# zxhuang1698/ShapeClipper

Measured on AMD Instinct MI355X. Metric: train-step images/sec (Pix3D cfg, bs32/GPU), higher is better.
Workload: dtype f32 (bf16x3-split MFMA, fp32 accumulate)

## Files before the change

include/shapeclipper_hip.h:

```cpp
#ifndef SHAPECLIPPER_HIP_H
#define SHAPECLIPPER_HIP_H
#include <stdint.h>
#ifdef __cplusplus
extern "C" {
#endif

int sc_chamfer3d_forward(const float* xyz1, const float* xyz2, float* dist1, float* dist2,
                         int32_t* idx1, int32_t* idx2, int b, int n, int m, void* stream);

int sc_chamfer3d_forward_split(const float* xyz1, const float* xyz2, float* dist1, float* dist2,
                               int32_t* idx1, int32_t* idx2, int b, int n, int m, int nsplit,
                               void* workspace, void* stream);

long long sc_chamfer3d_grid_workspace_bytes(int b, int n, int m);
int sc_chamfer3d_forward_grid(const float* xyz1, const float* xyz2, float* dist1, float* dist2,
                              int32_t* idx1, int32_t* idx2, int b, int n, int m, void* workspace, void* stream);

int sc_chamfer3d_backward(const float* xyz1, const float* xyz2, float* gradxyz1, float* gradxyz2,
                          const float* graddist1, const float* graddist2, const int32_t* idx1,
                          const int32_t* idx2, int b, int n, int m, void* stream);

long long sc_chamfer3d_backward_ordered_workspace_bytes(int b, int n, int m);
int sc_chamfer3d_backward_ordered_chunk(void);
int sc_chamfer3d_backward_ordered(const float* xyz1, const float* xyz2, float* gradxyz1, float* gradxyz2,
// ... 359 lines not shown
                            const float* flip_elev, const float* flip_theta, int n_images, float elev_lo, float elev_hi,
                            float theta_lo, float theta_hi, float margin_eps, int emd_p, float* out, float* grads,
                            void* stream);
int sc_camera_prior_backward(const float* grads, int n_images, const float* G_margin, const float* G_uniform,
                             const float* G_sym, float* g_azim, float* g_elev, float* g_theta, float* g_flip_azim,
                             float* g_flip_elev, float* g_flip_theta, void* stream);

int sc_transform_normal_forward(const float* normals, const float* pose, int n_images, int n_per_image, float* out,
                                void* stream);
int sc_transform_normal_backward(const float* normals, const float* g_out, int n_images, int n_per_image, float* g_pose,
                                 void* stream);

int sc_loss_total_forward(const float* const* values, const float* weights, int n_terms, float* total, unsigned char* bad,
                          void* stream);
int sc_loss_total_backward(const float* weights, int n_terms, const float* G, float* g_values, void* stream);

long long sc_conv3x3_pack_floats(int cin, int cout, int hw);
long long sc_conv3x3_workspace_floats(int hw);
int sc_conv3x3_tile_channels(int hw);
int sc_conv3x3_pack_multi(const long long* table, int n, float* dst, long long total, void* stream);
int sc_conv3x3_pack_multi_units(const long long* table, int n, float* dst, long long total, void* stream);
int sc_conv3x3_pack(const float* w, float* w_pack, int cin, int cout, int hw, int transpose_flip, void* stream);
int sc_conv3x3_forward(const float* x, const float* w_pack, float* out, float* workspace, int batch, int cin, int cout, int hw,
                       void* stream);

long long sc_conv3x3_pack_floats_split(int cin, int cout, int hw);
long long sc_conv3x3_workspace_floats_split(int hw);
int sc_conv3x3_tile_channels_split(int hw);
int sc_conv3x3_forward_split(const float* x, const float* w_pack, float* out, float* workspace, int batch, int cin, int cout, int hw,
                             void* stream);
int sc_conv3x3_forward_add(const float* x, const float* w_pack, const float* addend, float* out, float* workspace, int batch, int cin,
                           int cout, int hw, int split, void* stream);

long long sc_conv3x3s2_bd_pack_floats(int cin, int cout, int hw);
long long sc_conv3x3s2_bd_workspace_floats(int hw);
int sc_conv3x3s2_bd_pack(const float* w, float* w_pack, int cin, int cout, int hw, void* stream);
int sc_conv3x3s2_backward_data(const float* gy, const float* w_pack, float* gx, float* workspace, int batch, int cin, int cout, int hw,
                               void* stream);
int sc_conv3x3s2_wgrad(const float* gy, const float* x, float* dw, float* workspace, int batch, int cin, int cout, int hw, void* stream);
long long sc_conv3x3s2_pack_floats(int cin, int cout, int hw);
long long sc_conv3x3s2_workspace_floats(int hw);
int sc_conv3x3s2_forward(const float* x, const float* w_pack, float* out, float* workspace, int batch, int cin, int cout, int hw,
                         void* stream);

long long sc_conv3x3_wgrad_workspace_floats(int cin, int cout);
int sc_conv3x3_wgrad(const float* gy, const float* x, float* dw, float* workspace, int batch, int cin, int cout, int hw, void* stream);
int sc_conv3x3_wgrad_split(const float* gy, const float* x, float* dw, float* workspace, int batch, int cin, int cout, int hw, void* stream);

long long sc_conv_stem_wgrad_workspace_floats(void);
int sc_conv_stem_forward(const float* x, const float* w, float* out, int batch, void* stream);
int sc_conv_stem_wgrad(const float* gy, const float* x, float* dw, float* workspace, int batch, void* stream);

long long sc_conv1x1s2_wgrad_workspace_floats(int cin, int cout);
int sc_conv1x1s2_forward(const float* x, const float* w, float* out, int batch, int cin, int cout, int hin, void* stream);
int sc_conv1x1s2_backward_data(const float* gy, const float* w, float* gx, int batch, int cin, int cout, int hin, void* stream);
int sc_conv1x1s2_wgrad(const float* gy, const float* x, float* dw, float* workspace, int batch, int cin, int cout, int hin, void* stream);

typedef struct sc_block_args {
    const float *x, *pf1, *pf2, *pb1, *pb2;
    const float *g1, *b1, *g2, *b2;
    float *rm1, *rv1, *rm2, *rv2;
    int64_t *nt1, *nt2;
    float *y1, *a1, *y2, *out, *st1, *st2;
    float *conv_ws, *bn_ws, *wgrad_ws;
    const float* d_out;
    float *dy2, *dres, *da1, *dy1, *dx, *gw1, *gw2, *dgb1, *dgb2;
// ... 67 lines not shown
```

shapeclipper_amd/_lib.py:

```python
from __future__ import annotations

import ctypes
import os
import re
import threading
from typing import Optional

import torch

_HERE = os.path.dirname(os.path.abspath(__file__))
LIB_PATH = os.environ.get("SHAPECLIPPER_HIP_LIB") or os.path.join(_HERE, "lib", "libshapeclipper_hip.so")

HEADER_PATH = os.path.join(_HERE, os.pardir, "include", "shapeclipper_hip.h")
_CTYPES = {"int": ctypes.c_int, "long long": ctypes.c_longlong, "float": ctypes.c_float, "double": ctypes.c_double}


def read_signatures(text):
    text = re.sub(r"/\*.*?\*/|//[^\n]*", " ", text, flags=re.S)
    text = re.sub(r"^[ \t]*#.*$", " ", text, flags=re.M)
    text = re.sub(r"typedef struct sc_block_args \{.*?\} sc_block_args", " ", text, flags=re.S)
    text = re.sub(r'extern "C" \{|\}', " ", text)
    sigs = {}
    for decl in filter(None, (" ".join(d.split()) for d in text.split(";"))):
        m = re.fullmatch(r"(int|long long) (sc_\w+)\((.*)\)", decl)
        if m is None:
            raise RuntimeError("shapeclipper_amd: include/shapeclipper_hip.h: unrecognised declaration %r" % decl)
        params = [] if m.group(3) == "void" else m.group(3).split(",")
        try:
            args = [ctypes.c_void_p if "*" in p else _CTYPES[" ".join(w for w in p.split()[:-1] if w != "const")] for p in params]
        except KeyError:
            raise RuntimeError("shapeclipper_amd: include/shapeclipper_hip.h: unrecognised parameter type in %r" % decl) from None
        sigs[m.group(2)] = (_CTYPES[m.group(1)], args)
    return sigs


with open(HEADER_PATH) as _f:
    SIGNATURES = read_signatures(_f.read())
SYMBOLS = tuple(n for n, (res, _) in SIGNATURES.items() if res is ctypes.c_int)
SYMBOLS_OTHER = tuple(n for n, (res, _) in SIGNATURES.items() if res is ctypes.c_longlong)

_lib: Optional[ctypes.CDLL] = None

TIMING = None
TIMING_SKIP = ("sc_sdf_stream_pack", "sc_sdf_stream_pack_bytes", "sc_rgb_composite_backward_fused_parts", "sc_rgb_composite_backward_fused_partial_floats", "sc_latent_bias_forward", "sc_latent_bias_backward", "sc_set_reserved_cus", "sc_grid_cus", "sc_chamfer3d_backward_ordered_chunk","sc_conv3x3_release_tables", "sc_linear_bn_supported", "sc_linear_bn_forward", "sc_linear_bn_backward", "sc_linear_backward_data", "sc_bn_splits", "sc_isosurface_blocks_per_image", "sc_marching_cubes_mesh_vertex_blocks_per_image", "sc_bn_act_forward", "sc_bn_act_backward", "sc_bn_relu_pool_forward", "sc_bn_relu_pool_backward",
               "sc_conv3x3_forward", "sc_conv3x3_forward_split", "sc_conv3x3_forward_add", "sc_conv3x3_wgrad", "sc_conv3x3_wgrad_split", "sc_conv3x3_pack", "sc_conv3x3_pack_multi", "sc_conv3x3_pack_multi_units",
               "sc_conv_stem_forward", "sc_conv_stem_wgrad", "sc_conv1x1s2_forward", "sc_conv1x1s2_backward_data", "sc_conv1x1s2_wgrad",
               "sc_conv3x3s2_forward", "sc_conv3x3s2_bd_pack", "sc_conv3x3s2_backward_data", "sc_conv3x3s2_wgrad", "sc_conv3x3_tile_channels", "sc_conv3x3_tile_channels_split",
               "sc_basic_block_forward", "sc_basic_block_backward")

class _Timed:

    def __init__(self, name, fn):
        self.name, self.fn = name, fn

    def __call__(self, *args):
        if TIMING is None:
            return self.fn(*args)
        s, e = torch.cuda.Event(enable_timing=True), torch.cuda.Event(enable_timing=True)
        s.record()
        code = self.fn(*args)
        e.record()
        TIMING.setdefault(self.name, []).append((s, e, args))
        return code


class _LibProxy:

    def __init__(self, cdll):
        self._cdll = cdll
        for name, (restype, argtypes) in SIGNATURES.items():
            fn = getattr(cdll, name)
            fn.restype, fn.argtypes = restype, argtypes
            setattr(self, name, _Timed(name, fn) if restype is ctypes.c_int and name not in TIMING_SKIP else fn)


class HipLibraryMissing(RuntimeError):
    pass


def load():
    global _lib
# ... 43 lines not shown
```

shapeclipper_amd/csrc/conv3x3.hip:

```cpp
#include <hip/hip_runtime.h>

#include <map>
#include <mutex>
#include <tuple>
#include <vector>

#include "grid_cus.hpp"
#include "shapeclipper_hip.h"

#ifndef SC_CONV_SPANS
#define SC_CONV_SPANS 1
#endif
#ifndef SC_CONV_ABLATE
#define SC_CONV_ABLATE 0
#endif

namespace sc {

#ifdef SC_CONV_PROFILE
__device__ unsigned long long* conv_prof_buf = nullptr;
#define CV_STAMP(ID) { const unsigned long long t_ = __builtin_amdgcn_s_memrealtime(); if (conv_prof_buf && tid == 0) conv_prof_buf[(size_t)g * 32 + (ID)] = t_; }
#else
#define CV_STAMP(ID)
#endif

typedef float f32x16 __attribute__((ext_vector_type(16)));
typedef __bf16 cv_bf16x8 __attribute__((ext_vector_type(8)));
typedef __bf16 cv_bf16x2 __attribute__((ext_vector_type(2)));
typedef __attribute__((address_space(3))) void* lptr_cv_t;

__device__ __forceinline__ void conv_glds16(const void* gsrc, unsigned lds_dst) {
    unsigned keep;
    asm volatile("s_mov_b32 %0, m0\n\ts_mov_b32 m0, %2\n\ts_nop 0\n\tglobal_load_lds_dwordx4 %1, off\n\ts_mov_b32 m0, %0"
                 : "=&s"(keep) : "v"(gsrc), "s"(lds_dst) : "memory");
}

template <int W_, int CT_, int PT_, int WGM_, int WGN_, bool SPLIT_ = false, int S_ = 1, bool BD2_ = false>
struct ConvCfg {
    static constexpr int W = W_, CT = CT_, PT = PT_, WGM = WGM_, WGN = WGN_, CB = 8;
// ... 436 lines not shown
        for (int i = 0; i < C::WM; ++i)
#pragma unroll
            for (int j = 0; j < C::WN; ++j) {
                const float4 v = src[(((wave * C::WM + i) * C::WN + j) * 4 + (r0 >> 2)) * 64 + lane];
                acc[i][j][0] += v.x; acc[i][j][1] += v.y; acc[i][j][2] += v.z; acc[i][j][3] += v.w;
            }
    }
    const int tile = sp.rounds * G + t;
    int phase, pt, ct;
    conv_tile_decode<C>(tile, nct, phase, pt, ct);
#pragma unroll
    for (int j = 0; j < C::WN; ++j) {
        const int p = pt * C::PT + (wn * C::WN + j) * 32 + (lane & 31);
        if (p >= npix) continue;
        int cs;
        float* ob = conv_out_pixel<C>(out, p, phase, cout, cs);
#pragma unroll
        for (int i = 0; i < C::WM; ++i)
#pragma unroll
            for (int r = 0; r < 4; ++r) {
                const int co = ct * C::CT + (wm * C::WM + i) * 32 + r + 2 * r0 + 4 * (lane >> 5);
                if (co < cout) ob[(size_t)co * cs] = addend ? acc[i][j][r] + addend[(ob - out) + (size_t)co * cs] : acc[i][j][r];
            }
    }
#ifdef SC_CONV_PROFILE
    asm volatile("s_waitcnt vmcnt(0)" ::: "memory");
    if (conv_prof_buf && tid == 0) conv_prof_buf[(size_t)(8192 + blockIdx.x * 4 + blockIdx.y) * 2 + 1] = __builtin_amdgcn_s_memrealtime();
#endif
}

__device__ __forceinline__ float conv_w_at(const float* __restrict__ w, int cin, int cout, int co, int ci, int tap, int transpose_flip) {
    return transpose_flip ? w[((size_t)ci * cout + co) * 9 + (8 - tap)] : w[((size_t)co * cin + ci) * 9 + tap];
}
__device__ __forceinline__ unsigned conv_bf16_piece(float v, int pc) {
    const __bf16 h0 = (__bf16)v;
    const float r1 = v - (float)h0;
    const __bf16 h1 = (__bf16)r1;
    const __bf16 h2 = (__bf16)(r1 - (float)h1);
    const __bf16 h = pc == 0 ? h0 : pc == 1 ? h1 : h2;
    return (unsigned)__builtin_bit_cast(unsigned short, h);
}
__device__ __forceinline__ float conv_pack_word(const float* __restrict__ w, unsigned t, int CT, int nk, int cin, int cout, int flip,
                                                bool split) {
    if (!split) {
        const int s4 = (int)(t & 3);
        t >>= 2;
        const int cl = (int)(t % CT);
        t /= CT;
        const int h = (int)(t & 1);
        t >>= 1;
        const int tap = (int)(t % 9);
        t /= 9;
        const int kb = (int)(t % nk), ct = (int)(t / nk);
        const int ci = kb * 8 + 4 * h + s4, co = ct * CT + cl;
        return co < cout ? conv_w_at(w, cin, cout, co, ci, tap, flip) : 0.f;
    }
    const int wi = (int)(t & 3);
    t >>= 2;
    const int cl = (int)(t % CT);
    t /= CT;
    const int h = (int)(t & 1);
    t >>= 1;
    const int pc = (int)(t % 3);
    t /= 3;
    const int slot = (int)(t % 9);
    t /= 9;
    const int nkp = (nk + 1) >> 1, kp = (int)(t % nkp), ct = (int)(t / nkp);
    const int kb = 2 * kp + (slot < 4 ? 0 : (slot < 8 ? 1 : h)), tap = slot < 8 ? 2 * (slot & 3) + h : 8;
    const int co = ct * CT + cl, ci = kb * 8 + 2 * wi;
    unsigned lo = 0, hi = 0;
    if (kb < nk && co < cout) {
        lo = conv_bf16_piece(conv_w_at(w, cin, cout, co, ci, tap, flip), pc);
        hi = conv_bf16_piece(conv_w_at(w, cin, cout, co, ci + 1, tap, flip), pc);
    }
// ... 46 lines not shown
using Conv56S = ConvCfg<56, 64, 512, 1, 8, true>;
using Conv28S = ConvCfg<28, 64, 512, 1, 8, true>;
using Conv14S = ConvCfg<14, 64, 512, 1, 8, true>;
using Conv7S = ConvCfg<7, 64, 256, 1, 8, true>;
using Conv28BD = ConvCfg<28, 64, 512, 1, 8, true, 1, true>;
using Conv14BD = ConvCfg<14, 64, 512, 1, 8, true, 1, true>;
using Conv7BD = ConvCfg<7, 64, 256, 1, 8, true, 1, true>;

template <class C>
static long long pack_floats(int cin, int cout) {
    if (cin % C::CB) return -1;
    const long long nct = (cout + C::CT - 1) / C::CT, nk = cin / C::CB;
    return C::PAIRED ? nct * ((nk + 1) / 2) * 9 * C::PSZ : nct * nk * C::WIMG;
}

__global__ void conv3x3_pack_multi_kernel(const long long* __restrict__ table_g, int n, float* __restrict__ dst, long long total) {
    __shared__ long long table[128 * 6];
    for (int i = threadIdx.x; i < n * 6; i += blockDim.x) table[i] = table_g[i];
    __syncthreads();
    for (long long i = (long long)blockIdx.x * blockDim.x + threadIdx.x; i < total; i += (long long)gridDim.x * blockDim.x) {
        int lo = 0, hi = n - 1;
        while (lo < hi) {
            const int mid = (lo + hi + 1) >> 1;
            if (table[mid * 6 + 1] <= i) lo = mid; else hi = mid - 1;
        }
        const long long* row = table + lo * 6;
        const float* w = reinterpret_cast<const float*>(row[0]);
        const int cin = (int)row[2], cout = (int)row[3], CT = (int)row[4], flags = (int)row[5];
        dst[i] = conv_pack_word(w, (unsigned)(i - row[1]), CT, cin / 8, cin, cout, flags & 1, (flags & 2) != 0);
    }
}

__global__ __launch_bounds__(256) void conv3x3_pack_multi_split_kernel(const long long* __restrict__ table_g, int n, float* __restrict__ dst) {
    constexpr int CT = 64, UNIT = 9 * 3 * 2 * CT * 4, LST = 145;
    __shared__ float wl[CT * LST];
    __shared__ long long row_s[6];
    const int tid = threadIdx.x;
    const long long i0 = (long long)blockIdx.x * UNIT;
    if (tid == 0) {
        int lo = 0, hi = n - 1;
        while (lo < hi) {
            const int mid = (lo + hi + 1) >> 1;
            if (table_g[mid * 6 + 1] <= i0) lo = mid; else hi = mid - 1;
        }
        for (int k = 0; k < 6; ++k) row_s[k] = table_g[lo * 6 + k];
    }
    __syncthreads();
    const float* w = reinterpret_cast<const float*>(row_s[0]);
    const int cin = (int)row_s[2], cout = (int)row_s[3], flip = (int)row_s[5] & 1, nkp = (cin / 8 + 1) / 2;
    const int unit = (int)((i0 - row_s[1]) / UNIT), ct = unit / nkp, kp = unit - ct * nkp;
    for (int e = tid; e < 16 * CT * 9; e += 256) {
        int cl, sc, tap;
        float v = 0.f;
        if (flip) {
            sc = e / (CT * 9);
            const int r = e - sc * (CT * 9);
            cl = r / 9; tap = 8 - (r - cl * 9);
            if (ct * CT + cl < cout && kp * 16 + sc < cin) v = w[((size_t)(kp * 16 + sc) * cout + ct * CT) * 9 + r];
        } else {
            cl = e / 144;
            const int r = e - cl * 144;
            sc = r / 9; tap = r - sc * 9;
            if (ct * CT + cl < cout && kp * 16 + sc < cin) v = w[((size_t)(ct * CT + cl) * cin + kp * 16) * 9 + r];
        }
        wl[cl * LST + sc * 9 + tap] = v;
    }
    __syncthreads();
    for (int v = tid; v < UNIT; v += 256) {
        const int wi = v & 3, cl = (v >> 2) & 63, h = (v >> 8) & 1, q = v >> 9, pc = q % 3, slot = q / 3;
        const int kl = slot < 4 ? 0 : (slot < 8 ? 1 : h), tap = slot < 8 ? 2 * (slot & 3) + h : 8;
        const unsigned lo = conv_bf16_piece(wl[cl * LST + (8 * kl + 2 * wi) * 9 + tap], pc);
        const unsigned hi = conv_bf16_piece(wl[cl * LST + (8 * kl + 2 * wi + 1) * 9 + tap], pc);
        dst[i0 + v] = __uint_as_float(lo | (hi << 16));
    }
}

static int conv_grid() { return grid_cus(); }

template <class C>
static long long workspace_floats() { return (long long)conv_grid() * C::WGS_PER_CU * 2 * C::TILE; }

template <class C>
static int launch_pack(const float* w, float* wpack, int cin, int cout, int tf, hipStream_t st) {
    if (cin % C::CB) return (int)hipErrorInvalidValue;
    const long long total = pack_floats<C>(cin, cout);
    hipLaunchKernelGGL((conv3x3_pack_kernel<C>), dim3((unsigned)((total + 255) / 256 < 2048 ? (total + 255) / 256 : 2048)), dim3(256), 0, st,
                       w, wpack, cin, cout, tf);
    return (int)hipGetLastError();
}

struct SpanTable {
    int* dev = nullptr;
    std::vector<int> host;
};
static std::mutex span_mu;
static std::map<std::tuple<int, int, int, int, int>, SpanTable> span_cache;

static const int* conv_spans(int tail_tiles, int nk, int G, int ov2, hipStream_t st) {
    std::map<std::tuple<int, int, int, int, int>, SpanTable>& cache = span_cache;
    int dev = 0;
    (void)hipGetDevice(&dev);
    std::lock_guard<std::mutex> lock(span_mu);
    const auto key = std::make_tuple(dev, tail_tiles, nk, G, ov2);
// ... 253 lines not shown
```

shapeclipper_amd/model/resnet.py:

```python
from __future__ import annotations

import torch
import torch.nn as nn

from ..functional import basic_block, basic_block_takes, bn_act, bn_relu_maxpool, conv1x1s2, conv3x3, conv3x3s2, conv_stem

FUSED_BN = True
HIP_CONV3X3 = True
HIP_CONV_STEM = True
HIP_CONV3X3_S2 = True
HIP_CONV3X3_S2_GRADS = True
HIP_CONV_1X1 = True
FUSED_BLOCK = True
HIP_CONV3X3_SPLIT = True


class BasicBlock(nn.Module):
    expansion = 1

    def __init__(self, inplanes, planes, stride=1, downsample=None):
        super().__init__()
        self.conv1 = nn.Conv2d(inplanes, planes, 3, stride, 1, bias=False)
        self.bn1 = nn.BatchNorm2d(planes)
        self.relu = nn.ReLU(inplace=True)
# ... 52 lines not shown
        if not FUSED_BN:
            if groups > 1:
                return torch.cat([self.forward(c) for c in x.chunk(groups)], 0)
            x = self.maxpool(self.relu(self.bn1(self.conv1(x))))
            x = self.layer4(self.layer3(self.layer2(self.layer1(x))))
        else:
            use_hip = HIP_CONV3X3 if getattr(self, "hip_conv3x3", None) is None else self.hip_conv3x3
            packs = self._conv_packs(x) if use_hip else None
            x = bn_relu_maxpool(self.bn1, conv_stem(self.conv1, x) if HIP_CONV_STEM else self.conv1(x), groups=groups)
            for layer in (self.layer1, self.layer2, self.layer3, self.layer4):
                for block in layer:
                    x = block(x, groups=groups, packs=packs, hip_conv=use_hip)
        return self.fc(torch.flatten(self.avgpool(x), 1))


def _conv_packs(self, x):
    from .. import ops
    if not (x.is_cuda and x.dtype == torch.float32 and x.shape[2] == x.shape[3]):
        return None
    key = (x.shape[2], x.device.index, HIP_CONV3X3_SPLIT)
    cache = self.__dict__.setdefault("_pack_cache", {})
    packs = cache.get(key)
    if packs is None or (packs and packs.stale()):
        side = ((x.shape[2] + 2 * 3 - 7) // 2 + 1 + 2 - 3) // 2 + 1
        items = []
        for layer in (self.layer1, self.layer2, self.layer3, self.layer4):
            for block in layer:
                if block.conv1.stride == (2, 2):
                    side = (side + 2 - 3) // 2 + 1
                for conv in ((block.conv2,) if block.conv1.stride != (1, 1) else (block.conv1, block.conv2)):
                    if ops.conv3x3_supported((1, conv.in_channels, side, side), conv.weight.shape, conv.stride, conv.padding) and conv.bias is None:
                        items.append((conv.weight, side))
        packs = cache[key] = ops.Conv3x3PackSet(items, split=HIP_CONV3X3_SPLIT) if items else False
    if packs:
        packs.refresh()
    return packs or None


ResNet._conv_packs = _conv_packs

_LAYERS = {"resnet18": [2, 2, 2, 2], "resnet34": [3, 4, 6, 3]}


def build(name: str, pretrained: bool = False, allow_random: bool = False) -> ResNet:
    if name not in _LAYERS:
        raise NotImplementedError("encoder '%s' (available: %s)" % (name, sorted(_LAYERS)))
    net = ResNet(_LAYERS[name])
    if pretrained:
        try:
            import torchvision
            state = getattr(torchvision.models, name)(pretrained=True).state_dict()
        except Exception as e:
            msg = "ImageNet weights for %s could not be loaded (%s: %s)" % (name, type(e).__name__, e)
            if not allow_random:
                raise RuntimeError(msg + "; pass --arch.enc_pretrained! to train the ResNet trunks from a random "
                                         "initialisation, or --load/--resume a checkpoint") from e
            from ..utils.util import log
            log.warn("WARNING: " + msg + " -- %s starts from a RANDOM initialisation" % name)
        else:
            net.load_state_dict(state)
    return net
```

shapeclipper_amd/model/runner.py:

```python
from __future__ import annotations

import contextlib
import importlib
import os
import shutil
import time
from copy import deepcopy

import numpy as np
import torch
import tqdm

from ..data.pix3d import sample_rays_device
from ..parallel import FlatGradAllReduce, ModuleHolder
from ..utils import eval_3D, options, util
from ..utils.util import EasyDict as edict
from ..utils.util import cleanup, log, setup

try:
    from ..utils import util_vis
except Exception:
    util_vis = None


# ... 175 lines not shown
                if cat_samples[c] >= 1:
                    continue
                cat_samples[c] += 1
                sample = {}
                for key, value in batch.items():
                    if isinstance(value, torch.Tensor):
                        sample[key] = value[i].unsqueeze(0)
                    elif isinstance(value, dict):
                        sample[key] = {k: v[i].unsqueeze(0) for k, v in value.items()}
                    else:
                        raise NotImplementedError(key)
                self.viz_data.append(sample)

    def build_networks(self, opt):
        if _rank0(opt): log.info("building networks...")
        name = "pretrainer" if opt.pretrain else "graph"
        module = importlib.import_module("shapeclipper_amd.model.{}".format(name))
        dev = torch.device("cuda", opt.device) if isinstance(opt.device, int) else torch.device(opt.device)
        reserve = int(options.hip(opt, "reserve_cus") or 0)
        if dev.type == "cuda":
            from .. import ops
            ops.set_reserved_cus(reserve if opt.world_size > 1 else 0)
        self.graph = ModuleHolder(module.Graph(opt).to(dev))
        if opt.world_size > 1:
            self.reducer = FlatGradAllReduce(self.graph.module, opt.world_size,
                                             overlap=None if options.hip(opt, "overlap_allreduce") else False)

    def setup_optimizer(self, opt):
        if _rank0(opt): log.info("setting up optimizers...")
        kwargs = {k: (tuple(v) if k == "betas" else v) for k, v in opt.optim.params.items()}
        on_gpu = next(self.graph.parameters()).is_cuda
        if on_gpu and self.optimizer in (torch.optim.Adam, torch.optim.AdamW) and options.hip(opt, "fused_adam"):
            kwargs.setdefault("fused", True)
        full, view = [], []
        for k, v in self.graph.named_parameters():
            full.append(v)
            if "estimator" in k:
                view.append(v)
        self.optim_full = self.optimizer([dict(params=full, lr=opt.optim.lr)], **kwargs)
        self.optim_V = self.optimizer([dict(params=view, lr=opt.optim.lr)], **kwargs)
        self._guarded_step = bool(kwargs.get("fused")) and bool(options.hip(opt, "guarded_step"))

    def restore_checkpoint(self, opt, best=False, evaluate=False):
        epoch_start, iter_start = None, None
        if opt.resume:
            if _rank0(opt): log.info("resuming from previous checkpoint...")
            epoch_start, iter_start, self.best_val = util.restore_checkpoint(
                opt, self, resume=opt.resume, best=best if opt.data.dataset != "openimage" else False, evaluate=evaluate)
        elif opt.load is not None:
            if _rank0(opt): log.info("loading weights from checkpoint {}...".format(opt.load))
            epoch_start, iter_start, _ = util.restore_checkpoint(opt, self, load_name=opt.load)
        elif _rank0(opt):
            log.info("initializing weights from scratch...")
        self.epoch_start = epoch_start or 0
        self.iter_start = iter_start or 0

    def setup_visualizer(self, opt):
        if _rank0(opt) and opt.tb:
            try:
                from torch.utils.tensorboard import SummaryWriter
                self.tb = SummaryWriter(log_dir=opt.output_path, flush_secs=10)
            except Exception:
                log.info("tensorboard not available; scalar logging goes to stdout only")

    def train(self, opt):
        if _rank0(opt): log.title("TRAINING START")
        self.graph.module.estimator.reset_scales()
        self.timer = edict(start=time.time(), it_mean=None)
        self.iter_skip = self.iter_start % len(self.train_loader)
        self.it = self.iter_start
        if not opt.resume:
            self.best_val, self.best_ep = np.inf, 1
        if self.iter_start == 0 and _rank0(opt) and opt.freq.eval:
# ... 709 lines not shown
```

shapeclipper_amd/ops.py:

```python
from __future__ import annotations

import collections
import ctypes
import weakref

import torch

from . import _lib
from .packing import n_tiles

_SCRATCH = {}


def _scratch(tag, dev, n_floats):
    if dev.type != "cuda":
        raise RuntimeError(_lib.NO_CPU)
    key = (tag, dev.index, torch._C._cuda_getCurrentRawStream(dev.index))
    buf = _SCRATCH.get(key)
    if buf is None or buf.numel() < n_floats:
        buf = _SCRATCH[key] = torch.empty(n_floats, device=dev, dtype=torch.float32)
    return buf


SDF_SCRATCH_FLOATS = 256 * 8 * 5 * 1024
# ... 1131 lines not shown


def conv3x3s2_backward_data(gy, w, hw):
    lib = _lib.load()
    gy, w = _aligned(gy), _aligned(w)
    B, cout = gy.shape[0], gy.shape[1]
    cin = w.shape[1]
    n = lib.sc_conv3x3s2_bd_pack_floats(cin, cout, hw)
    if n < 0 or tuple(gy.shape[2:]) != (hw // 2, hw // 2) or w.shape[0] != cout:
        raise RuntimeError("shapeclipper_amd: sc_conv3x3s2_backward_data does not take gy %s with w %s" % (tuple(gy.shape), tuple(w.shape)))
    w_pack = torch.empty(n, device=gy.device, dtype=torch.float32)
    _lib.check(lib.sc_conv3x3s2_bd_pack(_lib.ptr(w), _lib.ptr(w_pack), cin, cout, hw, _lib.stream()), "sc_conv3x3s2_bd_pack")
    ws = _scratch("conv s2bd %d" % hw, gy.device, lib.sc_conv3x3s2_bd_workspace_floats(hw))
    gx = torch.empty(B, cin, hw, hw, device=gy.device, dtype=torch.float32)
    _lib.check(lib.sc_conv3x3s2_backward_data(_lib.ptr(gy), _lib.ptr(w_pack), _lib.ptr(gx), _lib.ptr(ws), B, cin, cout, hw, _lib.stream()),
               "sc_conv3x3s2_backward_data")
    return gx


def conv3x3s2_backward_weight(gy, x):
    lib = _lib.load()
    gy, x = _aligned(gy), _aligned(x)
    B, cin, hw, _ = x.shape
    cout = gy.shape[1]
    n = lib.sc_conv3x3_wgrad_workspace_floats(cin, cout)
    if n < 0 or hw not in (56, 28, 14) or tuple(gy.shape) != (B, cout, hw // 2, hw // 2):
        raise RuntimeError("shapeclipper_amd: sc_conv3x3s2_wgrad does not take gy %s with x %s" % (tuple(gy.shape), tuple(x.shape)))
    ws = _scratch("conv wgrad", x.device, n)
    dw = torch.empty(cout, cin, 3, 3, device=x.device, dtype=torch.float32)
    _lib.check(lib.sc_conv3x3s2_wgrad(_lib.ptr(gy), _lib.ptr(x), _lib.ptr(dw), _lib.ptr(ws), B, cin, cout, hw, _lib.stream()), "sc_conv3x3s2_wgrad")
    return dw


class Conv3x3PackSet:

    def __init__(self, items, split=False):
        lib = _lib.load()
        self.split = bool(split)
        self.weights = [w for w, _ in items]
        self.ptrs = [w.data_ptr() for w in self.weights]
        rows, off, self.where = [], 0, {}
        for k, (w, side) in enumerate(items):
            if not (w.is_cuda and w.is_contiguous() and w.dtype == torch.float32):
                raise RuntimeError("shapeclipper_amd: Conv3x3PackSet needs contiguous fp32 device filters")
            for flip in (0, 1):
                cin, cout = (w.shape[0], w.shape[1]) if flip else (w.shape[1], w.shape[0])
                n = (lib.sc_conv3x3_pack_floats_split if split else lib.sc_conv3x3_pack_floats)(cin, cout, side)
                if n < 0:
                    raise RuntimeError("shapeclipper_amd: sc_conv3x3 does not take %dx%d maps with a %s filter" % (side, side, tuple(w.shape)))
                ct = (lib.sc_conv3x3_tile_channels_split if split else lib.sc_conv3x3_tile_channels)(side)
                rows.append([w.data_ptr(), off, cin, cout, ct, flip | (2 if split else 0)])
                self.where[(k, flip)] = (off, n)
                off += n
        if len(rows) > 128:
            raise RuntimeError("shapeclipper_amd: Conv3x3PackSet holds at most 64 filters (sc_conv3x3_pack_multi table limit)")
        dev = self.weights[0].device
        self.total = off
        self.units = bool(split) and all(r[4] == 64 for r in rows) and off % 13824 == 0
        self.table = torch.tensor(rows, dtype=torch.int64).to(dev)
        self.buf = torch.empty(off, device=dev, dtype=torch.float32)
        self.index = {id(w): k for k, w in enumerate(self.weights)}

    def stale(self):
        return any(w.data_ptr() != p for w, p in zip(self.weights, self.ptrs))

    def refresh(self):
        lib = _lib.load()
        fn = lib.sc_conv3x3_pack_multi_units if self.units else lib.sc_conv3x3_pack_multi
        _lib.check(fn(_lib.ptr(self.table), len(self.where), _lib.ptr(self.buf), self.total, _lib.stream()), "sc_conv3x3_pack_multi")

    def get(self, w, flip):
        off, n = self.where[(self.index[id(w)], int(flip))]
        return self.buf[off:off + n]


def linear_bn_supported(N, Cin, Cout, groups) -> bool:
    return bool(_lib.load().sc_linear_bn_supported(N, Cin, Cout, groups))


def linear_bn_forward(x, w, gamma, beta, res, running_mean, running_var, n_tracked, training, momentum, eps, relu, groups):
    N, Cin = x.shape
    Cout = w.shape[0]
    y, out = torch.empty(N, Cout, device=x.device, dtype=torch.float32), torch.empty(N, Cout, device=x.device, dtype=torch.float32)
    stats = torch.empty(2, groups, Cout, device=x.device, dtype=torch.float32)
    code = _lib.load().sc_linear_bn_forward(_lib.ptr(x), _lib.ptr(w), _lib.ptr(gamma), _lib.ptr(beta), _lib.ptr(res), _lib.ptr(y), _lib.ptr(out),
                                            _lib.ptr(stats[0]), _lib.ptr(stats[1]), _lib.ptr(running_mean), _lib.ptr(running_var), _lib.ptr(n_tracked),
                                            N, Cin, Cout, groups, 1 if training else 0, 1 if relu else 0,
                                            eps, momentum, _lib.stream())
    _lib.check(code, "sc_linear_bn_forward")
    return out, y, stats


def linear_bn_backward(g_out, gy_next, w_next, g_add, out, y, stats, gamma, x, want_res, training, relu, groups):
    N, Cin = x.shape
    Cout = y.shape[1]
    f32 = dict(device=x.device, dtype=torch.float32)
    gy = torch.empty(N, Cout, **f32)
# ... 828 lines not shown
```

shapeclipper_amd/utils/options.py:

```python
from __future__ import annotations

import collections
import importlib
import os
import random
import string
import sys

import numpy as np
import torch
import yaml

from . import util
from .util import EasyDict as edict
from .util import log

torch.backends.cudnn.benchmark = False

Switch = collections.namedtuple("Switch", ["key", "default", "kind", "text", "drives"])
HIP_TABLE = tuple(Switch(*row) for row in (
    ("device_rng", False, bool, "draw the render's jitter on the GPU (no 4 MB upload per render, another random stream than the reference)", None),
    ("device_choice", True, bool, "pick the regularisation view on the device (reg.n_views = 1)", None),
    ("device_rays", True, bool, "Pix3D: silhouette-weighted ray choice for the whole batch on the GPU (csrc/silhouette_rays.hip)", None),
    ("device_clip_preprocess", True, bool, "Pix3D: CLIP preprocessing on the GPU (csrc/clip_preprocess.hip)", None),
    ("fused_backward", True, bool, "SDF reverse pass with the weight gradients formed in the kernel (sc_sdf_backward_fused)", None),
    ("deterministic_conv", False, bool, "torch.backends.cudnn.deterministic, process-global", None),
    ("fused_loss", True, bool, "the render losses of one render in a single launch (csrc/loss.hip)", None),
    ("fused_adam", True, bool, "torch's fused Adam on the device", None),
    ("guarded_step", True, bool, "a non-finite loss skips the update on the device; the host raises one step later", None),
    ("batched_encoders", True, bool, "one grouped encoder pass and one grouped estimator pass per step", None),
    ("two_streams", True, bool, "the view estimator runs on a side stream next to the encoders", None),
    ("overlap_allreduce", False, bool, "multi-GPU: the early gradient segment is all-reduced from inside backward", None),
    ("reserve_cus", 0, (0, None), "multi-GPU: persistent convolution grids sized for the device's CUs minus this many", None),
    ("fused_block", True, bool, "one autograd node per stride-1 BasicBlock", ("model.resnet", "FUSED_BLOCK")),
    ("fused_bottleneck", True, bool, "1x1 Bottleneck_Linear blocks as fused launches (csrc/bottleneck.hip)", ("model.view_estimator", "HIP_BOTTLENECK")),
    ("fused_rgb_wgrad", True, bool, "RGB reverse pass forms the weight gradients in the kernel; off: Gy_l / r_l through HBM and sc_wgrad",
     ("ops", "FUSED_RGB_WGRAD")),
    ("rgb_stash", True, bool, "RGB forward parks its hidden activations for the reverse pass; off: the reverse pass recomputes them",
     ("ops", "RGB_STASH")),
    ("value_split", True, bool, "value-only SDF calls (evaluation grid) on the pre-split bf16x3 chain; off: fp32 MFMA", ("ops", "SDF_VALUE_SPLIT")),
    ("rgb_split", True, bool, "RGB network of the forward pass from pre-split bf16x3 fragments; off: fp32 MFMA", ("ops", "RGB_FWD_SPLIT")),
    ("rgb_bwd_split", True, bool, "RGB reverse chain from pre-split transposed fragments; off: fp32 MFMA (see HIP_REQUIRES)",
     ("ops", "RGB_BWD_SPLIT")),
    ("sdf_stream", True, bool, "SDF forward (value, feature, d sdf/dx) from streamed pre-split fragments; off: fp32 MFMA", ("ops", "SDF_FWD_STREAM")),
    ("upload_stream", True, bool, "the CPU-generator draws are copied on a stream of their own, ahead of the render",
     ("model.renderer", "UPLOAD_STREAM")),
    ("rocblas", True, bool, "the small fp32 GEMMs left to torch go through rocBLAS, process-global; off leaves torch's choice alone", None),
    ("conv3x3", True, bool, "3x3 stride-1 trunk convolutions on csrc/conv3x3.hip", ("model.resnet", "HIP_CONV3X3")),
    ("conv3x3_split", True, bool, "... as exact three-piece bf16 operand splits; off: fp32 MFMA throughout", ("model.resnet", "HIP_CONV3X3_SPLIT")),
    ("conv_stem", True, bool, "the 7x7 stride-2 stem convolution on its HIP kernel", ("model.resnet", "HIP_CONV_STEM")),
    ("conv1x1", True, bool, "the 1x1 stride-2 shortcut convolutions on their HIP kernels", ("model.resnet", "HIP_CONV_1X1")),
    ("conv3x3s2", True, bool, "the 3x3 stride-2 convolutions' forward on its HIP kernel", ("model.resnet", "HIP_CONV3X3_S2")),
    ("conv3x3s2_grads", True, bool, "... and their backward-data / weight gradient", ("model.resnet", "HIP_CONV3X3_S2_GRADS")),
    ("train_vis", False, bool, "training-time visualisation on rank 0: turn-table GIFs and periodic dumps", None),
    ("mesh_color", False, bool, "every mesh dump also writes a coloured PLY with vertex normals", None),
    ("largest_component", False, bool, "evaluation keeps the largest connected component of the level grid", None),
    ("surface_render", False, bool, "every per-sample dump also gets a render at the SDF zero crossing (Renderer.render_surface)", None),
    ("surface_refine", 3, (0, 16), "... refinement rounds of the crossing", None),
    ("surface_scale", 1, (1, 4), "... pixels per pixel side", None),
))
HIP = {row.key: row for row in HIP_TABLE}
# ... 228 lines not shown
```

Baseline: 1032.

## Fuse Adam update with conv3x3 filter repacking in one native launch

Replaces torch's fused Adam with a custom HIP kernel that updates all parameters in one launch. For conv3x3 filters it also writes the bf16x3-split packed weight images (forward and transposed) straight from the updated values. Pack sets are then marked current, so the per-step separate repack pass is skipped. The cost is a more complex pointer table with a pinned-memory upload ring, version tracking for pack staleness, and an Adam update computed in mixed double/float arithmetic that may differ slightly from torch's.

```diff
diff --git a/include/shapeclipper_hip.h b/include/shapeclipper_hip.h
--- a/include/shapeclipper_hip.h
+++ b/include/shapeclipper_hip.h
@@ -415,6 +415,9 @@
 int sc_conv3x3_forward_add(const float* x, const float* w_pack, const float* addend, float* out, float* workspace, int batch, int cin,
                            int cout, int hw, int split, void* stream);
 
+int sc_adam_step(const long long* tensors, int n_tensors, const long long* blocks, int n_blocks, const long long* chunks, int n_chunks,
+                 double lr, double beta1, double beta2, double eps, const float* found_inf, void* stream);
+
 long long sc_conv3x3s2_bd_pack_floats(int cin, int cout, int hw);
 long long sc_conv3x3s2_bd_workspace_floats(int hw);
 int sc_conv3x3s2_bd_pack(const float* w, float* w_pack, int cin, int cout, int hw, void* stream);
diff --git a/shapeclipper_amd/_lib.py b/shapeclipper_amd/_lib.py
--- a/shapeclipper_amd/_lib.py
+++ b/shapeclipper_amd/_lib.py
@@ -46,7 +46,8 @@
                "sc_conv3x3_forward", "sc_conv3x3_forward_split", "sc_conv3x3_forward_add", "sc_conv3x3_wgrad", "sc_conv3x3_wgrad_split", "sc_conv3x3_pack", "sc_conv3x3_pack_multi", "sc_conv3x3_pack_multi_units",
                "sc_conv_stem_forward", "sc_conv_stem_wgrad", "sc_conv1x1s2_forward", "sc_conv1x1s2_backward_data", "sc_conv1x1s2_wgrad",
                "sc_conv3x3s2_forward", "sc_conv3x3s2_bd_pack", "sc_conv3x3s2_backward_data", "sc_conv3x3s2_wgrad", "sc_conv3x3_tile_channels", "sc_conv3x3_tile_channels_split",
-               "sc_basic_block_forward", "sc_basic_block_backward")
+               "sc_basic_block_forward", "sc_basic_block_backward",
+               "sc_adam_step")
 
 class _Timed:
 
diff --git a/shapeclipper_amd/csrc/adam.hip b/shapeclipper_amd/csrc/adam.hip
--- /dev/null
+++ b/shapeclipper_amd/csrc/adam.hip
@@ -0,0 +1,193 @@
+#include <hip/hip_runtime.h>
+
+#include <cstdint>
+
+#include "conv_pack.hpp"
+#include "shapeclipper_hip.h"
+
+namespace sc {
+namespace adam {
+
+constexpr int THREADS = 1024, WAVES = THREADS / 64, CHUNK = 1024, TROW = 6, BROW = 8, CROW = 2;
+constexpr int FB = 64, SEG = FB * 9, LST = SEG + 1;
+constexpr int LDS_BYTES = FB * LST * 4;
+
+struct Coef {
+    float step_size, bc2_sqrt;
+    double b1, b2, eps;
+};
+
+__device__ __forceinline__ double pow_n(double b, unsigned n) {
+    double r = 1.0;
+    for (; n; n >>= 1, b *= b)
+        if (n & 1) r *= b;
+    return r;
+}
+
+__device__ __forceinline__ Coef coefficients(float step_old, double lr, double b1, double b2, double eps) {
+    const unsigned n = (unsigned)(step_old + 1.f);
+    const float bc1 = (float)(1.0 - pow_n(b1, n)), bc2_sqrt = (float)sqrt(1.0 - pow_n(b2, n));
+    return {(float)(lr / (double)bc1), bc2_sqrt, b1, b2, eps};
+}
+
+__device__ __forceinline__ void update(float& p, float g, float& m, float& v, const Coef& c) {
+    m = (float)fma(c.b1, (double)m, (1.0 - c.b1) * (double)g);
+    v = (float)fma(c.b2, (double)v, (1.0 - c.b2) * (double)g * (double)g);
+    const float denom = (float)((double)(sqrtf(v) / c.bc2_sqrt) + c.eps);
+    p -= c.step_size * m / denom;
+}
+
+__device__ __forceinline__ void update4(float4& p, const float4& g, float4& m, float4& v, const Coef& c) {
+    update(p.x, g.x, m.x, v.x, c);
+    update(p.y, g.y, m.y, v.y, c);
+    update(p.z, g.z, m.z, v.z, c);
+    update(p.w, g.w, m.w, v.w, c);
+}
+
+__device__ __forceinline__ float4 load4(const float* a, bool vec) {
+    if (vec) return *reinterpret_cast<const float4*>(a);
+    return make_float4(a[0], a[1], a[2], a[3]);
+}
+__device__ __forceinline__ void store4(float* a, const float4& x, bool vec) {
+    if (vec) {
+        *reinterpret_cast<float4*>(a) = x;
+    } else {
+        a[0] = x.x; a[1] = x.y; a[2] = x.z; a[3] = x.w;
+    }
+}
+__device__ __forceinline__ bool aligned16(const void* a, const void* b, const void* c, const void* d) {
+    return (((uintptr_t)a | (uintptr_t)b | (uintptr_t)c | (uintptr_t)d) & 15) == 0;
+}
+
+__global__ __launch_bounds__(THREADS) void adam_step_kernel(const long long* __restrict__ tensors, int n_tensors,
+                                                            const long long* __restrict__ blocks, int n_blocks,
+                                                            const long long* __restrict__ chunks, int n_chunks, double lr, double b1,
+                                                            double b2, double eps, const float* __restrict__ found_inf) {
+    extern __shared__ __attribute__((aligned(16))) float wl[];
+    const int tid = threadIdx.x;
+    const bool skip = found_inf != nullptr && *found_inf != 0.f;
+    if ((int)blockIdx.x >= n_blocks) {
+        const int wave = __builtin_amdgcn_readfirstlane(tid >> 6), lane = tid & 63;
+        const long long c = (long long)((int)blockIdx.x - n_blocks) * WAVES + wave;
+        if (skip || c >= n_chunks) return;
+        const int t = (int)chunks[c * CROW];
+        if (t < 0 || t >= n_tensors) return;
+        const long long start = chunks[c * CROW + 1];
+        const long long* tr = tensors + (size_t)t * TROW;
+        const long long left = tr[5] - start;
+        const int n = left < CHUNK ? (int)left : CHUNK;
+        float* __restrict__ p = reinterpret_cast<float*>(tr[0]) + start;
+        const float* __restrict__ g = reinterpret_cast<const float*>(tr[1]) + start;
+        float* __restrict__ m = reinterpret_cast<float*>(tr[2]) + start;
+        float* __restrict__ v = reinterpret_cast<float*>(tr[3]) + start;
+        const Coef cf = coefficients(*reinterpret_cast<const float*>(tr[4]), lr, b1, b2, eps);
+        const int nq = aligned16(p, g, m, v) ? n >> 2 : 0;
+#pragma unroll 1
+        for (int k0 = 0; k0 < 4 && 64 * k0 < nq; k0 += 2) {
+            float4 P[2], G[2], M[2], V[2];
+#pragma unroll
+            for (int k = 0; k < 2; ++k) {
+                const int q = lane + 64 * (k0 + k);
+                if (q < nq) {
+                    P[k] = load4(p + 4 * q, true); G[k] = load4(g + 4 * q, true);
+                    M[k] = load4(m + 4 * q, true); V[k] = load4(v + 4 * q, true);
+                }
+            }
+#pragma unroll
+            for (int k = 0; k < 2; ++k) {
+                const int q = lane + 64 * (k0 + k);
+                if (q < nq) {
+                    update4(P[k], G[k], M[k], V[k], cf);
+                    store4(p + 4 * q, P[k], true); store4(m + 4 * q, M[k], true); store4(v + 4 * q, V[k], true);
+                }
+            }
+        }
+        for (int e = 4 * nq + lane; e < n; e += 64) {
+            float pe = p[e], me = m[e], ve = v[e];
+            update(pe, g[e], me, ve, cf);
+            p[e] = pe; m[e] = me; v[e] = ve;
+        }
+        return;
+    }
+    const long long* br = blocks + (size_t)blockIdx.x * BROW;
+    const int t = (int)br[0], bi = (int)br[1], bj = (int)br[2], cin = (int)br[3], cout = (int)br[4];
+    if (t < 0 || t >= n_tensors || (bi + 1) * FB > cout || (bj + 1) * FB > cin) return;
+    const long long* tr = tensors + (size_t)t * TROW;
+    if (tr[5] != (long long)cin * cout * 9) return;
+    const size_t base = ((size_t)bi * FB * cin + (size_t)bj * FB) * 9, rs = (size_t)cin * 9;
+    float* __restrict__ p = reinterpret_cast<float*>(tr[0]) + base;
+    const float* __restrict__ g = reinterpret_cast<const float*>(tr[1]) + base;
+    float* __restrict__ m = reinterpret_cast<float*>(tr[2]) + base;
+    float* __restrict__ v = reinterpret_cast<float*>(tr[3]) + base;
+    const bool vec = aligned16(p, g, m, v);
+    Coef cf = {};
+    if (!skip) cf = coefficients(*reinterpret_cast<const float*>(tr[4]), lr, b1, b2, eps);
+    for (int q = tid; q < FB * (SEG / 4); q += THREADS) {
+        const int cl = q / (SEG / 4), r = 4 * (q - cl * (SEG / 4));
+        const size_t off = cl * rs + r;
+        float4 P = load4(p + off, vec);
+        if (!skip) {
+            const float4 G = load4(g + off, vec);
+            float4 M = load4(m + off, vec), V = load4(v + off, vec);
+            update4(P, G, M, V, cf);
+            store4(p + off, P, vec); store4(m + off, M, vec); store4(v + off, V, vec);
+        }
+        float* w = wl + cl * LST + r;
+        w[0] = P.x; w[1] = P.y; w[2] = P.z; w[3] = P.w;
+    }
+    __syncthreads();
+    float* __restrict__ buf = reinterpret_cast<float*>(br[7]);
+    const long long unit_f = br[5] + ((long long)bi * (cin / 16) + 4 * bj) * CONV_UNIT;
+    const long long unit_b = br[6] + ((long long)bj * (cout / 16) + 4 * bi) * CONV_UNIT;
+    for (int u = tid; u < 8 * (CONV_UNIT / 3); u += THREADS) {
+        const int wi = u & 3, cl = (u >> 2) & 63, h = (u >> 8) & 1, r = u >> 9, un = r / 9, slot = r - 9 * un, j = un & 3;
+        int kl, tap;
+        conv_unit_slot(slot, h, kl, tap);
+        const int sc = 16 * j + 8 * kl + 2 * wi;
+        float lo, hi;
+        float* dst;
+        if (un < 4) {
+            lo = wl[cl * LST + sc * 9 + tap]; hi = wl[cl * LST + (sc + 1) * 9 + tap];
+            dst = buf + unit_f + (long long)j * CONV_UNIT;
+        } else {
+            lo = wl[sc * LST + cl * 9 + 8 - tap]; hi = wl[(sc + 1) * LST + cl * 9 + 8 - tap];
+            dst = buf + unit_b + (long long)j * CONV_UNIT;
+        }
+        unsigned a[3], b[3];
+        conv_bf16_split(lo, a);
+        conv_bf16_split(hi, b);
+        const int w0 = (slot * 6 + h) * 256 + cl * 4 + wi;
+#pragma unroll
+        for (int pc = 0; pc < 3; ++pc) dst[w0 + pc * 512] = __uint_as_float(a[pc] | (b[pc] << 16));
+    }
+}
+
+__global__ void adam_advance_kernel(const long long* __restrict__ tensors, int n_tensors, const float* __restrict__ found_inf) {
+    const int i = blockIdx.x * blockDim.x + threadIdx.x;
+    if (i >= n_tensors || (found_inf != nullptr && *found_inf != 0.f)) return;
+    float* step = reinterpret_cast<float*>(tensors[(size_t)i * TROW + 4]);
+    *step += 1.f;
+}
+
+}
+}
+
+extern "C" int sc_adam_step(const long long* tensors, int n_tensors, const long long* blocks, int n_blocks, const long long* chunks,
+                            int n_chunks, double lr, double beta1, double beta2, double eps, const float* found_inf, void* stream) {
+    using namespace sc::adam;
+    if (n_tensors <= 0) return 0;
+    if (n_blocks < 0 || n_chunks < 0 || !tensors || (n_blocks && !blocks) || (n_chunks && !chunks)) return (int)hipErrorInvalidValue;
+    const long long grid = (long long)n_blocks + (n_chunks + WAVES - 1) / WAVES;
+    if (grid > 0x7fffffffLL) return (int)hipErrorInvalidValue;
+    if (grid) {
+        const int lds = n_blocks ? LDS_BYTES : 0;
+        if (lds) (void)hipFuncSetAttribute((const void*)adam_step_kernel, hipFuncAttributeMaxDynamicSharedMemorySize, LDS_BYTES);
+        hipLaunchKernelGGL(adam_step_kernel, dim3((unsigned)grid), dim3(THREADS), lds, (hipStream_t)stream, tensors, n_tensors, blocks, n_blocks,
+                           chunks, n_chunks, lr, beta1, beta2, eps, found_inf);
+        const int code = (int)hipGetLastError();
+        if (code) return code;
+    }
+    hipLaunchKernelGGL(adam_advance_kernel, dim3((unsigned)((n_tensors + 255) / 256)), dim3(256), 0, (hipStream_t)stream, tensors, n_tensors,
+                       found_inf);
+    return (int)hipGetLastError();
+}
diff --git a/shapeclipper_amd/csrc/conv3x3.hip b/shapeclipper_amd/csrc/conv3x3.hip
--- a/shapeclipper_amd/csrc/conv3x3.hip
+++ b/shapeclipper_amd/csrc/conv3x3.hip
@@ -5,6 +5,7 @@
 #include <tuple>
 #include <vector>
 
+#include "conv_pack.hpp"
 #include "grid_cus.hpp"
 #include "shapeclipper_hip.h"
 
@@ -507,14 +508,6 @@
 __device__ __forceinline__ float conv_w_at(const float* __restrict__ w, int cin, int cout, int co, int ci, int tap, int transpose_flip) {
     return transpose_flip ? w[((size_t)ci * cout + co) * 9 + (8 - tap)] : w[((size_t)co * cin + ci) * 9 + tap];
 }
-__device__ __forceinline__ unsigned conv_bf16_piece(float v, int pc) {
-    const __bf16 h0 = (__bf16)v;
-    const float r1 = v - (float)h0;
-    const __bf16 h1 = (__bf16)r1;
-    const __bf16 h2 = (__bf16)(r1 - (float)h1);
-    const __bf16 h = pc == 0 ? h0 : pc == 1 ? h1 : h2;
-    return (unsigned)__builtin_bit_cast(unsigned short, h);
-}
 __device__ __forceinline__ float conv_pack_word(const float* __restrict__ w, unsigned t, int CT, int nk, int cin, int cout, int flip,
                                                 bool split) {
     if (!split) {
@@ -627,7 +620,7 @@
 }
 
 __global__ __launch_bounds__(256) void conv3x3_pack_multi_split_kernel(const long long* __restrict__ table_g, int n, float* __restrict__ dst) {
-    constexpr int CT = 64, UNIT = 9 * 3 * 2 * CT * 4, LST = 145;
+    constexpr int CT = 64, UNIT = CONV_UNIT, LST = 145;
     __shared__ float wl[CT * LST];
     __shared__ long long row_s[6];
     const int tid = threadIdx.x;
@@ -663,7 +656,8 @@
     __syncthreads();
     for (int v = tid; v < UNIT; v += 256) {
         const int wi = v & 3, cl = (v >> 2) & 63, h = (v >> 8) & 1, q = v >> 9, pc = q % 3, slot = q / 3;
-        const int kl = slot < 4 ? 0 : (slot < 8 ? 1 : h), tap = slot < 8 ? 2 * (slot & 3) + h : 8;
+        int kl, tap;
+        conv_unit_slot(slot, h, kl, tap);
         const unsigned lo = conv_bf16_piece(wl[cl * LST + (8 * kl + 2 * wi) * 9 + tap], pc);
         const unsigned hi = conv_bf16_piece(wl[cl * LST + (8 * kl + 2 * wi + 1) * 9 + tap], pc);
         dst[i0 + v] = __uint_as_float(lo | (hi << 16));
diff --git a/shapeclipper_amd/csrc/conv_pack.hpp b/shapeclipper_amd/csrc/conv_pack.hpp
--- /dev/null
+++ b/shapeclipper_amd/csrc/conv_pack.hpp
@@ -0,0 +1,27 @@
+#pragma once
+#include <hip/hip_runtime.h>
+
+namespace sc {
+
+__device__ __forceinline__ void conv_bf16_split(float v, unsigned (&h)[3]) {
+    const __bf16 h0 = (__bf16)v;
+    const float r1 = v - (float)h0;
+    const __bf16 h1 = (__bf16)r1;
+    const __bf16 h2 = (__bf16)(r1 - (float)h1);
+    h[0] = (unsigned)__builtin_bit_cast(unsigned short, h0);
+    h[1] = (unsigned)__builtin_bit_cast(unsigned short, h1);
+    h[2] = (unsigned)__builtin_bit_cast(unsigned short, h2);
+}
+__device__ __forceinline__ unsigned conv_bf16_piece(float v, int pc) {
+    unsigned h[3];
+    conv_bf16_split(v, h);
+    return pc == 0 ? h[0] : pc == 1 ? h[1] : h[2];
+}
+
+constexpr int CONV_UNIT = 9 * 3 * 2 * 64 * 4;
+__device__ __forceinline__ void conv_unit_slot(int slot, int h, int& kl, int& tap) {
+    kl = slot < 4 ? 0 : (slot < 8 ? 1 : h);
+    tap = slot < 8 ? 2 * (slot & 3) + h : 8;
+}
+
+}
diff --git a/shapeclipper_amd/model/resnet.py b/shapeclipper_amd/model/resnet.py
--- a/shapeclipper_amd/model/resnet.py
+++ b/shapeclipper_amd/model/resnet.py
@@ -108,7 +108,7 @@
                     if ops.conv3x3_supported((1, conv.in_channels, side, side), conv.weight.shape, conv.stride, conv.padding) and conv.bias is None:
                         items.append((conv.weight, side))
         packs = cache[key] = ops.Conv3x3PackSet(items, split=HIP_CONV3X3_SPLIT) if items else False
-    if packs:
+    if packs and not packs.is_current():
         packs.refresh()
     return packs or None
 
diff --git a/shapeclipper_amd/model/runner.py b/shapeclipper_amd/model/runner.py
--- a/shapeclipper_amd/model/runner.py
+++ b/shapeclipper_amd/model/runner.py
@@ -231,13 +231,16 @@
         on_gpu = next(self.graph.parameters()).is_cuda
         if on_gpu and self.optimizer in (torch.optim.Adam, torch.optim.AdamW) and options.hip(opt, "fused_adam"):
             kwargs.setdefault("fused", True)
+        cls = self.optimizer
+        if kwargs.get("fused") and cls is torch.optim.Adam and os.environ.get("SC_TORCH_FUSED_ADAM", "0") in ("", "0"):
+            from ..optim import Adam as cls
         full, view = [], []
         for k, v in self.graph.named_parameters():
             full.append(v)
             if "estimator" in k:
                 view.append(v)
-        self.optim_full = self.optimizer([dict(params=full, lr=opt.optim.lr)], **kwargs)
-        self.optim_V = self.optimizer([dict(params=view, lr=opt.optim.lr)], **kwargs)
+        self.optim_full = cls([dict(params=full, lr=opt.optim.lr)], **kwargs)
+        self.optim_V = cls([dict(params=view, lr=opt.optim.lr)], **kwargs)
         self._guarded_step = bool(kwargs.get("fused")) and bool(options.hip(opt, "guarded_step"))
 
     def restore_checkpoint(self, opt, best=False, evaluate=False):
diff --git a/shapeclipper_amd/ops.py b/shapeclipper_amd/ops.py
--- a/shapeclipper_amd/ops.py
+++ b/shapeclipper_amd/ops.py
@@ -1187,6 +1187,18 @@
     return dw
 
 
+_PACK_SETS = weakref.WeakSet()
+_PACK_SET_GENERATION = 0
+
+
+def pack_sets():
+    return list(_PACK_SETS)
+
+
+def pack_set_generation():
+    return _PACK_SET_GENERATION
+
+
 class Conv3x3PackSet:
 
     def __init__(self, items, split=False):
@@ -1215,9 +1227,19 @@
         self.table = torch.tensor(rows, dtype=torch.int64).to(dev)
         self.buf = torch.empty(off, device=dev, dtype=torch.float32)
         self.index = {id(w): k for k, w in enumerate(self.weights)}
+        self.current = None
+        global _PACK_SET_GENERATION
+        _PACK_SETS.add(self)
+        _PACK_SET_GENERATION += 1
 
     def stale(self):
         return any(w.data_ptr() != p for w, p in zip(self.weights, self.ptrs))
+
+    def mark_current(self):
+        self.current = [w._version for w in self.weights]
+
+    def is_current(self):
+        return self.current is not None and self.current == [w._version for w in self.weights] and not self.stale()
 
     def refresh(self):
         lib = _lib.load()
diff --git a/shapeclipper_amd/optim.py b/shapeclipper_amd/optim.py
--- /dev/null
+++ b/shapeclipper_amd/optim.py
@@ -0,0 +1,156 @@
+from __future__ import annotations
+
+import operator
+
+import numpy as np
+import torch
+
+from . import _lib
+
+CHUNK = 1024
+BLOCK = 64
+TROW, BROW, CROW = 6, 8, 2
+RING = 4
+
+
+def plan(sizes, filters):
+    blocks, chunks = [], []
+    for t, n in enumerate(sizes):
+        if t in filters:
+            cout, cin = filters[t]
+            if cout % BLOCK or cin % BLOCK or cout * cin * 9 != n:
+                raise ValueError("shapeclipper_amd: filter %d [%d, %d, 3, 3] with %d elements cannot be cut into 64 x 64 blocks" % (t, cout, cin, n))
+            bi, bj = np.divmod(np.arange((cout // BLOCK) * (cin // BLOCK), dtype=np.int64), cin // BLOCK)
+            blocks.append(np.stack([np.full_like(bi, t), bi, bj], 1))
+        elif n > 0:
+            start = np.arange(0, n, CHUNK, dtype=np.int64)
+            chunks.append(np.stack([np.full_like(start, t), start], 1))
+    return (np.concatenate(blocks) if blocks else np.zeros((0, 3), np.int64),
+            np.concatenate(chunks) if chunks else np.zeros((0, 2), np.int64))
+
+
+class _Table:
+
+    def __init__(self, params, state, sets):
+        from . import ops
+        self.params, self.sets = params, sets
+        self.generation = ops.pack_set_generation()
+        self.m = [state[p]["exp_avg"] for p in params]
+        self.v = [state[p]["exp_avg_sq"] for p in params]
+        self.steps = [state[p]["step"] for p in params]
+        index = {id(p): t for t, p in enumerate(params)}
+        filters, where = {}, {}
+        for s in sets:
+            for k, w in enumerate(s.weights):
+                filters[index[id(w)]] = (w.shape[0], w.shape[1])
+                where[index[id(w)]] = (s.where[(k, 0)][0], s.where[(k, 1)][0], s.buf.data_ptr())
+        blocks, chunks = plan([p.numel() for p in params], filters)
+        self.n_tensors, self.n_blocks, self.n_chunks = len(params), len(blocks), len(chunks)
+        rows = np.zeros((self.n_blocks, BROW), np.int64)
+        for b, (t, bi, bj) in enumerate(blocks.tolist()):
+            cout, cin = filters[t]
+            rows[b] = (t, bi, bj, cin, cout) + where[t]
+        static = np.concatenate([rows.ravel(), chunks.ravel()])
+        dev = params[0].device
+        self.static = torch.from_numpy(static).to(dev) if static.size else torch.zeros(1, dtype=torch.int64, device=dev)
+        self.blocks_ptr = self.static.data_ptr()
+        self.chunks_ptr = self.blocks_ptr + 8 * rows.size
+        self.dev = torch.empty(self.n_tensors, TROW, dtype=torch.int64, device=dev)
+        self.ring = []
+        for _ in range(RING):
+            host = torch.empty(self.n_tensors, TROW, dtype=torch.int64).pin_memory()
+            view = host.numpy()
+            view[:, 2] = [t.data_ptr() for t in self.m]
+            view[:, 3] = [t.data_ptr() for t in self.v]
+            view[:, 4] = [t.data_ptr() for t in self.steps]
+            view[:, 5] = [p.numel() for p in params]
+            self.ring.append([host, view, None])
+        self.ptrs, self.turn = None, 0
+
+    def upload(self, ptrs):
+        slot = self.ring[self.turn % RING]
+        self.turn += 1
+        host, view, copied = slot
+        if copied is not None:
+            copied.synchronize()
+        view[:, 0], view[:, 1] = ptrs[0::2], ptrs[1::2]
+        self.dev.copy_(host, non_blocking=True)
+        slot[2] = torch.cuda.Event()
+        slot[2].record()
+        self.ptrs = ptrs
+
+
+class Adam(torch.optim.Adam):
+
+    def _native_group(self, group):
+        return (group["weight_decay"] == 0 and not group["amsgrad"] and not group["maximize"] and not group.get("capturable")
+                and not group.get("differentiable") and not group.get("decoupled_weight_decay") and isinstance(group["lr"], (int, float))
+                and isinstance(group["betas"][0], (int, float)) and isinstance(group["betas"][1], (int, float)))
+
+    def _native_build(self, live):
+        from . import ops
+        dev = live[0].device
+        for p in live:
+            g = p.grad
+            if not (p.is_cuda and p.device == dev and p.dtype == torch.float32 and p.is_contiguous() and g.layout == torch.strided
+                    and g.dtype == torch.float32 and g.is_contiguous() and g.device == dev):
+                return None
+        fresh = [p for p in live if len(self.state[p]) == 0]
+        if fresh:
+            steps = torch.zeros(len(fresh), dtype=torch.float32, device=dev)
+            for k, p in enumerate(fresh):
+                self.state[p].update(step=steps[k], exp_avg=torch.zeros_like(p, memory_format=torch.preserve_format),
+                                     exp_avg_sq=torch.zeros_like(p, memory_format=torch.preserve_format))
+        for p in live:
+            st = self.state[p]
+            if not all(k in st and torch.is_tensor(st[k]) and st[k].is_cuda and st[k].dtype == torch.float32 and st[k].is_contiguous()
+                       for k in ("step", "exp_avg", "exp_avg_sq")) or st["exp_avg"].shape != p.shape or st["exp_avg_sq"].shape != p.shape:
+                return None
+        ids, claimed, sets = {id(p) for p in live}, set(), []
+        for s in ops.pack_sets():
+            if (s.units and not s.stale() and s.buf.device == dev and all(id(w) in ids and id(w) not in claimed for w in s.weights)
+                    and all(w.shape[0] % BLOCK == 0 and w.shape[1] % BLOCK == 0 for w in s.weights)):
+                sets.append(s)
+                claimed.update(id(w) for w in s.weights)
+        return _Table(live, self.state, sets)
+
+    @torch.no_grad()
+    def step(self, closure=None):
+        from . import ops
+        found_inf = getattr(self, "found_inf", None)
+        if (closure is not None or getattr(self, "grad_scale", None) is not None or not all(self._native_group(g) for g in self.param_groups)
+                or not (found_inf is None or (found_inf.is_cuda and found_inf.dtype == torch.float32 and found_inf.numel() == 1))):
+            return super().step(closure)
+        if "_native_tables" not in self.__dict__:
+            self._native_tables = {}
+            self.register_load_state_dict_post_hook(lambda opt: opt._native_tables.clear())
+        work = []
+        for gi, group in enumerate(self.param_groups):
+            live, ptrs = [], []
+            for p in group["params"]:
+                g = p.grad
+                if g is not None:
+                    live.append(p)
+                    ptrs.append(p.data_ptr())
+                    ptrs.append(g.data_ptr())
+            if not live:
+                continue
+            table = self._native_tables.get(gi)
+            if (table is None or table.generation != ops.pack_set_generation() or len(live) != len(table.params)
+                    or not all(map(operator.is_, live, table.params)) or any(s.stale() for s in table.sets)):
+                table = self._native_tables[gi] = self._native_build(live)
+                if table is None:
+                    del self._native_tables[gi]
+                    return super().step(closure)
+            work.append((group, table, ptrs))
+        lib = _lib.load()
+        for group, table, ptrs in work:
+            if ptrs != table.ptrs:
+                table.upload(ptrs)
+            _lib.check(lib.sc_adam_step(_lib.ptr(table.dev), table.n_tensors, table.blocks_ptr, table.n_blocks, table.chunks_ptr, table.n_chunks,
+                                        group["lr"], group["betas"][0], group["betas"][1], group["eps"], _lib.ptr(found_inf), _lib.stream()),
+                       "sc_adam_step")
+            torch.autograd.graph.increment_version(table.params)
+            for s in table.sets:
+                s.mark_current()
+        return None
diff --git a/shapeclipper_amd/utils/options.py b/shapeclipper_amd/utils/options.py
--- a/shapeclipper_amd/utils/options.py
+++ b/shapeclipper_amd/utils/options.py
@@ -26,7 +26,7 @@
     ("fused_backward", True, bool, "SDF reverse pass with the weight gradients formed in the kernel (sc_sdf_backward_fused)", None),
     ("deterministic_conv", False, bool, "torch.backends.cudnn.deterministic, process-global", None),
     ("fused_loss", True, bool, "the render losses of one render in a single launch (csrc/loss.hip)", None),
-    ("fused_adam", True, bool, "torch's fused Adam on the device", None),
+    ("fused_adam", True, bool, "Adam in one native launch that also writes the trunks' filter images (torch's fused kernel for what it does not take)", None),
     ("guarded_step", True, bool, "a non-finite loss skips the update on the device; the host raises one step later", None),
     ("batched_encoders", True, bool, "one grouped encoder pass and one grouped estimator pass per step", None),
     ("two_streams", True, bool, "the view estimator runs on a side stream next to the encoders", None),
```

New measurement: 1043 (median of 4 runs). No clear change (+1.1%).
